# Virtana/robot_camera_calibration

Measured on NVIDIA B200. Metric: BA corner observations/s (residual+Jacobian+normal equations), higher is better.
Workload: dtype f64

## Files before the change

### robot_camera_calibration_b200/csrc/assemble.cu

```cuda
#include "common.cuh"
#include "kernels.h"
#include "model.cuh"

namespace rcc {

template <bool RIG, bool EPASS, bool OWN_IS_VIEW>
struct RowSink {
  using PG = PassGeom<RIG>;
  double* row[2];
  double w;
  __device__ __forceinline__ void put6(int i, int col, const double* v) {
    double2* d = reinterpret_cast<double2*>(row[i] + col);
    d[0] = make_double2(w * v[0], w * v[1]);
    d[1] = make_double2(w * v[2], w * v[3]);
    d[2] = make_double2(w * v[4], w * v[5]);
  }
  __device__ __forceinline__ void shared(int i, const double* js, double r) {
    double2* d = reinterpret_cast<double2*>(row[i] + 6);
    d[0] = make_double2(w * js[0], w * js[1]);
    d[1] = make_double2(w * js[2], w * js[3]);
    d[2] = make_double2(w * js[4], w * js[5]);
    d[3] = make_double2(w * js[6], w * js[7]);
    d[4] = make_double2(w * js[8], w * r);
  }
  __device__ __forceinline__ void marker(int i, const double* jm) {
    if (!OWN_IS_VIEW) put6(i, 0, jm);
    else if (EPASS) put6(i, PG::COL_C, jm);
  }
  __device__ __forceinline__ void view(int i, const double* jv) {
    if (OWN_IS_VIEW) put6(i, 0, jv);
    else if (EPASS) put6(i, PG::COL_C, jv);
  }
  __device__ __forceinline__ void ext(int i, const double* jx) { put6(i, PG::COL_X, jx); }
};

__device__ __forceinline__ void cp_async16(void* smem_dst, const void* gmem_src) {
  const unsigned d = (unsigned)__cvta_generic_to_shared(smem_dst);
  asm volatile("cp.async.ca.shared.global [%0], [%1], 16;" ::"r"(d), "l"(gmem_src) : "memory");
}
__device__ __forceinline__ void cp_async_commit() { asm volatile("cp.async.commit_group;" ::: "memory"); }
__device__ __forceinline__ void cp_async_wait_all() { asm volatile("cp.async.wait_group 0;" ::: "memory"); }

__device__ __forceinline__ void dmma(double (&c)[2], double a, double b) {
  asm volatile("mma.sync.aligned.m8n8k4.row.col.f64.f64.f64.f64 {%0,%1}, {%2}, {%3}, {%0,%1};"
               : "+d"(c[0]), "+d"(c[1])
               : "d"(a), "d"(b));
}

#ifndef RCC_K2_MIN_CTAS
#define RCC_K2_MIN_CTAS 3
#endif
#ifndef RCC_K2_MIN_CTAS_F
#define RCC_K2_MIN_CTAS_F 3
#endif

template <bool RIG, bool EPASS>
struct WarpSmem {
  using PG = PassGeom<RIG>;
  static constexpr int RS = EPASS ? PG::RS_E : PG::RS_F;
  static constexpr int BS = 8 * RS + 2;
  static constexpr int STAGE = PG::BPW * BS;
  static constexpr int CONSTS = STAGE + 2 * PG::BPW * POSEX;
  static constexpr int TOTAL = CONSTS + 2 * POSEX + 16;
};

template <bool RIG, bool EPASS, bool OWN_IS_VIEW, bool LOSS>
__global__ void __launch_bounds__(PassGeom<RIG>::WARPS * 32,
                                  (RIG && EPASS) ? 2 : ((!RIG && !EPASS) ? RCC_K2_MIN_CTAS_F : RCC_K2_MIN_CTAS))
assemble_kernel(const AssembleArgs a) {
  using PG = PassGeom<RIG>;
  using WS = WarpSmem<RIG, EPASS>;
  constexpr int BPW = PG::BPW, RS = WS::RS, BS = WS::BS;
  constexpr int PART = EPASS ? PG::PART_E : PG::PART_F;
  extern __shared__ __align__(16) double smem[];
  const int warp = threadIdx.x >> 5, lane = threadIdx.x & 31;
  const int launch_pos = blockIdx.x * PG::WARPS + warp;
  if (launch_pos >= a.n_chunks) return;
  const int chunk_id = a.chunk_list ? a.chunk_list[launch_pos] : launch_pos;
  double* wsm = smem + warp * WS::TOTAL;
  double* rows = wsm;
  double* stage = wsm + WS::STAGE;
  double* own_x = wsm + WS::CONSTS;
  double* ext_x = own_x + POSEX;
  double* sh = ext_x + POSEX;

  const Chunk ch = a.chunks[chunk_id];
  const int b = lane >> 2;
  const int t = lane & 3;
  const double* oth_table = OWN_IS_VIEW ? a.marker_x : a.view_x;

  {
    const double* src = (OWN_IS_VIEW ? a.view_x : a.marker_x) + (size_t)ch.own * POSEX;
    if (lane < POSEX) own_x[lane] = src[lane];
    if (RIG && lane < POSEX) ext_x[lane] = a.ext_x[(size_t)ch.cam * POSEX + lane];
    if (lane < PG::SP) sh[lane] = a.shared[ch.cam * PG::SP + lane];
    for (int k = lane; k < BPW * BS; k += 32) rows[k] = 0.0;
  }
  auto load_oth = [&](int it) -> int {
    return (lane < BPW && it + lane < ch.count) ? a.oth[(int64_t)ch.start + it + lane] : 0;
  };
  auto issue_stage = [&](int it, int buf, int oth_reg) {
    constexpr int PIECES = BPW * (POSEX / 2);
#pragma unroll
    for (int r = 0; r < PIECES / 32; ++r) {
      const int idx = lane + 32 * r;
      const int q = idx / (POSEX / 2), c = idx - q * (POSEX / 2);
      const int o = __shfl_sync(0xffffffffu, oth_reg, q);
      if (it + q < ch.count)
        cp_async16(stage + (buf * BPW + q) * POSEX + 2 * c, oth_table + (size_t)o * POSEX + 2 * c);
    }
    cp_async_commit();
  };
  int oth_cur = load_oth(0);
  int oth_nxt = load_oth(BPW);
  issue_stage(0, 0, oth_cur);
  double2 px_nxt = make_double2(0.0, 0.0);
  if (b < ch.count) px_nxt = *reinterpret_cast<const double2*>(a.pix + ((int64_t)ch.start + b) * 8 + 2 * t);

  double cAA[2] = {0.0, 0.0}, cAB[2] = {0.0, 0.0}, cBB[2] = {0.0, 0.0};
  double cAX[2] = {0.0, 0.0}, cBX[2] = {0.0, 0.0}, cXX[2] = {0.0, 0.0};
  double cost_acc = 0.0;
  double* my_rows = rows + b * BS + t * RS;
  const double* frag = rows + (lane & 3) * RS + (lane >> 2);
  int buf = 0;

  for (int it = 0; it < ch.count; it += BPW, buf ^= 1) {
    const bool valid = (it + b) < ch.count;
    const int64_t g = (int64_t)ch.start + it + b;
    cp_async_wait_all();
    __syncwarp();
    const double2 px = px_nxt;
    if (it + BPW < ch.count) {
      issue_stage(it + BPW, buf ^ 1, oth_nxt);
      oth_nxt = load_oth(it + 2 * BPW);
      if (it + BPW + b < ch.count) px_nxt = *reinterpret_cast<const double2*>(a.pix + (g + BPW) * 8 + 2 * t);
    }
    const double* ox_rec = stage + (buf * BPW + b) * POSEX;
    const double* vx = OWN_IS_VIEW ? own_x : ox_rec;
    const double* mx = OWN_IS_VIEW ? ox_rec : own_x;
    BlockGeom<RIG> geo;
    double ox = 0.0, oy = 0.0;
    if (valid) {
      block_geometry<RIG>(vx, mx, RIG ? ext_x : nullptr, geo);
      corner_xy(t, mx[PX_HS], ox, oy);
    }
    double w = 1.0;
    if (LOSS) {
      double s_blk = 0.0;
      if (valid) {
        CornerRows<RIG> c;
        eval_corner<RIG, false>(geo, sh, ox, oy, px.x, px.y, c);
        s_blk = c.r[0] * c.r[0] + c.r[1] * c.r[1];
      }
      s_blk += __shfl_xor_sync(0xffffffffu, s_blk, 1);
      s_blk += __shfl_xor_sync(0xffffffffu, s_blk, 2);
      double rho1;
      const double rho = robust_rho(a.loss, a.loss_a2, s_blk, rho1);
      w = sqrt(rho1);
      if (EPASS && valid && t == 0) cost_acc += rho;
    }
    if (valid) {
      RowSink<RIG, EPASS, OWN_IS_VIEW> sink{{my_rows, my_rows + 4 * RS}, w};
      double r0, r1;
      const double depth = eval_corner_emit<RIG>(geo, sh, ox, oy, px.x, px.y, sink, r0, r1);
      if (!(depth > 0.0) || !isfinite(r0) || !isfinite(r1)) *a.fail_flag = 1;
    }
    __syncwarp();
    auto block_products = [&](int bb) {
      const double* f0 = frag + bb * BS;
      const double* f1 = f0 + 4 * RS;
      const double a0 = f0[0], a1 = f1[0];
      const double b0 = f0[PG::COL_B], b1 = f1[PG::COL_B];
      dmma(cAA, a0, a0); dmma(cAA, a1, a1);
      dmma(cAB, a0, b0); dmma(cAB, a1, b1);
      if (EPASS) { dmma(cBB, b0, b0); dmma(cBB, b1, b1); }
      if (RIG) {
        const double x0 = f0[PG::COL_X], x1 = f1[PG::COL_X];
        dmma(cAX, a0, x0); dmma(cAX, a1, x1);
        if (EPASS) {
          dmma(cBX, b0, x0); dmma(cBX, b1, x1);
          dmma(cXX, x0, x0); dmma(cXX, x1, x1);
        }
      }
      if (EPASS) {
        const double t0 = f0[PG::COL_C], t1 = f1[PG::COL_C];
        double cW[2] = {0.0, 0.0};
        dmma(cW, a0, t0); dmma(cW, a1, t1);
        if (lane < 24 && (lane & 3) < 3)
          *reinterpret_cast<double2*>(a.W + ((int64_t)ch.start + it + bb) * 36 + (lane >> 2) * 6 + 2 * (lane & 3)) =
              make_double2(cW[0], cW[1]);
      }
    };
    if (ch.count - it >= BPW) {
#pragma unroll
      for (int bb = 0; bb < BPW; ++bb) block_products(bb);
    } else {
#pragma unroll 1
      for (int bb = 0; bb < ch.count - it; ++bb) block_products(bb);
    }
    __syncwarp();
  }

  double2* out = reinterpret_cast<double2*>(a.partials + (size_t)chunk_id * PART) + lane;
  if (EPASS) {
    out[TE_AA * 32] = make_double2(cAA[0], cAA[1]);
    out[TE_AB * 32] = make_double2(cAB[0], cAB[1]);
    out[TE_BB * 32] = make_double2(cBB[0], cBB[1]);
    if (RIG) {
      out[TE_AX * 32] = make_double2(cAX[0], cAX[1]);
      out[TE_BX * 32] = make_double2(cBX[0], cBX[1]);
      out[TE_XX * 32] = make_double2(cXX[0], cXX[1]);
    }
    if (LOSS) {
#pragma unroll
      for (int o = 16; o > 0; o >>= 1) cost_acc += __shfl_xor_sync(0xffffffffu, cost_acc, o);
    }
    if (lane == 0) a.partials[(size_t)chunk_id * PART + PG::TILES_E * 64] = cost_acc;
  } else {
    out[TF_AA * 32] = make_double2(cAA[0], cAA[1]);
    out[TF_AB * 32] = make_double2(cAB[0], cAB[1]);
    if (RIG) out[TF_AX * 32] = make_double2(cAX[0], cAX[1]);
  }
}

template <bool RIG, bool EPASS, bool OWN_IS_VIEW, bool LOSS>
static void launch_assemble_t(const AssembleArgs& a, cudaStream_t s) {
  using PG = PassGeom<RIG>;
  if (a.n_chunks == 0) return;
  const size_t smem = PG::WARPS * WarpSmem<RIG, EPASS>::TOTAL * sizeof(double);
  auto k = assemble_kernel<RIG, EPASS, OWN_IS_VIEW, LOSS>;
  static SmemOptIn optin;
  optin.ensure(k, smem);
  const int grid = ceil_div(a.n_chunks, PG::WARPS);
  k<<<grid, PG::WARPS * 32, smem, s>>>(a);
  RCC_CUDA(cudaGetLastError());
}

template <bool LOSS>
static void launch_assemble_l(bool rig, bool epass, bool own_is_view, const AssembleArgs& a, cudaStream_t s) {
  const int sel = (rig ? 4 : 0) | (epass ? 2 : 0) | (own_is_view ? 1 : 0);
  switch (sel) {
    case 0: launch_assemble_t<false, false, false, LOSS>(a, s); break;
    case 1: launch_assemble_t<false, false, true, LOSS>(a, s); break;
    case 2: launch_assemble_t<false, true, false, LOSS>(a, s); break;
    case 3: launch_assemble_t<false, true, true, LOSS>(a, s); break;
    case 4: launch_assemble_t<true, false, false, LOSS>(a, s); break;
    case 5: launch_assemble_t<true, false, true, LOSS>(a, s); break;
    case 6: launch_assemble_t<true, true, false, LOSS>(a, s); break;
    default: launch_assemble_t<true, true, true, LOSS>(a, s); break;
  }
}

// ... 218 lines not shown
```

### robot_camera_calibration_b200/csrc/evaluate.cu

```cuda
#include "common.cuh"
#include "kernels.h"
#include "model.cuh"

namespace rcc {

constexpr int EVAL_THREADS = 256;
constexpr int EVAL_CTAS_PER_SM = 2;

int eval_grid(int64_t n) {
  const int64_t groups = (n + 7) / 8;
  return (int)std::max<int64_t>(1, std::min<int64_t>((groups + EVAL_THREADS / 32 - 1) / (EVAL_THREADS / 32),
                                                     (int64_t)NUM_SMS_B200 * EVAL_CTAS_PER_SM));
}

__device__ __forceinline__ double block_sum(double v, double* red) {
#pragma unroll
  for (int o = 16; o > 0; o >>= 1) v += __shfl_xor_sync(0xffffffffu, v, o);
  const int warp = threadIdx.x >> 5, lane = threadIdx.x & 31;
  if (lane == 0) red[warp] = v;
  __syncthreads();
  double s = 0.0;
  if (threadIdx.x == 0) {
    for (int w = 0; w < (int)(blockDim.x >> 5); ++w) s += red[w];
  }
// ... 92 lines not shown
  }
  const double s = block_sum(cost, red);
  if (threadIdx.x == 0 && a.cost2_partials) a.cost2_partials[blockIdx.x] = s;
}

template <bool RIG>
static void launch_evaluate_t(const EvalArgs& a, cudaStream_t s) {
  evaluate_kernel<RIG><<<eval_grid(a.n), EVAL_THREADS, 0, s>>>(a);
  RCC_CUDA(cudaGetLastError());
}

template <bool RIG, bool OWN_IS_VIEW>
struct CeresSink {
  using ER = EvalRec<RIG>;
  double* rec;
  int q, t;
  double d0[5];
  __device__ __forceinline__ void put6(int off, int i, const double* v) {
    double2* d = reinterpret_cast<double2*>(rec + off + q * 48 + (2 * t + i) * 6);
    d[0] = make_double2(v[0], v[1]);
    d[1] = make_double2(v[2], v[3]);
    d[2] = make_double2(v[4], v[5]);
  }
  __device__ __forceinline__ void shared(int i, const double* js, double r) {
    double2* d = reinterpret_cast<double2*>(rec + ER::JI + q * 32 + (2 * t + i) * 4);
    d[0] = make_double2(js[0], js[1]);
    d[1] = make_double2(js[2], js[3]);
    rec[ER::RES + q * 8 + 2 * t + i] = r;
    if (i == 0) {
#pragma unroll
      for (int k = 0; k < 5; ++k) d0[k] = js[4 + k];
    } else {
      d = reinterpret_cast<double2*>(rec + ER::JD + q * 40 + 10 * t);
      d[0] = make_double2(d0[0], d0[1]);
      d[1] = make_double2(d0[2], d0[3]);
      d[2] = make_double2(d0[4], js[4]);
      d[3] = make_double2(js[5], js[6]);
      d[4] = make_double2(js[7], js[8]);
    }
  }
  __device__ __forceinline__ void marker(int i, const double* jm) { put6(ER::JM, i, jm); }
  __device__ __forceinline__ void view(int i, const double* jv) { put6(ER::JV, i, jv); }
  __device__ __forceinline__ void ext(int i, const double* jx) { put6(ER::JX, i, jx); }
};

__device__ __forceinline__ void ev_cp_async16(void* smem_dst, const void* gmem_src) {
// ... 187 lines not shown
```

### robot_camera_calibration_b200/csrc/kernels.h

```cpp
#pragma once

#include <cuda_runtime.h>
#include <math.h>
#include <stdint.h>

namespace rcc {

template <bool RIG>
struct PassGeom {
  static constexpr int BPW = 8;
  static constexpr int SP = RIG ? 15 : 9;
  static constexpr int WARPS = 4;
  static constexpr int RS_E = RIG ? 36 : 28;
  static constexpr int RS_F = RIG ? 28 : 20;
  static constexpr int COL_B = 8, COL_X = 16, COL_C = RIG ? 24 : 16;
  static constexpr int TILES_E = RIG ? 6 : 3;
  static constexpr int TILES_F = RIG ? 3 : 2;
  static constexpr int PART_E = TILES_E * 64 + 8;
  static constexpr int PART_F = TILES_F * 64;
};
enum TileE : int { TE_AA = 0, TE_AB = 1, TE_BB = 2, TE_AX = 3, TE_BX = 4, TE_XX = 5 };
enum TileF : int { TF_AA = 0, TF_AB = 1, TF_AX = 2 };

struct Chunk {
  int32_t own;
  int32_t cam;
  int32_t start;
  int32_t count;
};

struct AssembleArgs {
  const int32_t* oth;
  const double* pix;
  const Chunk* chunks;
  int32_t n_chunks;
  const int32_t* chunk_list;
  const double* view_x;
  const double* marker_x;
  const double* ext_x;
  const double* shared;
  double* partials;
  double* W;
  int32_t* fail_flag;
  int32_t loss;
  double loss_a2;
};

void launch_assemble(bool rig, bool epass, bool own_is_view, const AssembleArgs& a, cudaStream_t s);

struct FinalizeSideArgs {
  const double* partials;
  const Chunk* chunks;
  const int32_t* chunk_ptr;
  int32_t n_own;
  int32_t n_shared;
  double* Hoo;
  double* go;
  double* Hos;
};

struct FinalizeSharedArgs {
  const double* part_e;
  const int32_t* cam_chunks_e;
  const int32_t* cam_ptr_e;
  int32_t n_cam;
  int32_t n_shared;
  double* Hss;
  double* gs;
// ... 209 lines not shown
```

### robot_camera_calibration_b200/csrc/model.cuh

```cuda
#pragma once

#include <math.h>

#if defined(__CUDACC__)
#define RCC_HD __host__ __device__ __forceinline__
#else
#define RCC_HD inline
#endif

namespace rcc {

constexpr int POSEX = 24;
constexpr int PX_R = 0, PX_JR = 9, PX_T = 18;
constexpr int PX_RJ = PX_JR;
constexpr int PX_HS = 21;

RCC_HD double sinc_d(double t2, double t) {
  if (t2 < 1e-6) return 1.0 - t2 * (1.0 / 6.0) + t2 * t2 * (1.0 / 120.0);
  return sin(t) / t;
}

RCC_HD void expand_pose(const double* __restrict__ p, double* __restrict__ o) {
  const double x = p[0], y = p[1], z = p[2];
  const double t2 = x * x + y * y + z * z;
// ... 199 lines not shown
  if (!RIG) {
    a_cross(A, P, 1.0, B);
#pragma unroll
    for (int i = 0; i < 2; ++i) row_mat(B[i], g.Jrv, out.jv[i]);
  } else {
    double qb[3], Ax[2][3];
#pragma unroll
    for (int i = 0; i < 3; ++i) qb[i] = g.Rbm[3 * i] * ox + g.Rbm[3 * i + 1] * oy + g.qb0[i];
#pragma unroll
    for (int i = 0; i < 2; ++i) {
      row_mat(A[i], g.RxT, Ax[i]);
#pragma unroll
      for (int j = 0; j < 3; ++j) out.jx[i][3 + j] = -Ax[i][j];
    }
    a_cross(Ax, qb, 1.0, B);
#pragma unroll
    for (int i = 0; i < 2; ++i) row_mat(B[i], g.Jrv, out.jv[i]);
    a_cross(A, P, 1.0, B);
#pragma unroll
    for (int i = 0; i < 2; ++i) row_mat(B[i], g.Jrx, out.jx[i]);
  }
}

template <bool RIG, class Geo, class Sink>
RCC_HD double eval_corner_emit(const Geo& g, const double* __restrict__ sh, double ox, double oy,
                               double pu, double pv, Sink& sink, double& r0, double& r1) {
  const double fx = sh[0], fy = sh[1], cx = sh[2], cy = sh[3];
  const double k1 = sh[4], k2 = sh[5], p1 = sh[6], p2 = sh[7], k3 = sh[8];
  double d[3], P[3];
#pragma unroll
  for (int i = 0; i < 3; ++i) {
    d[i] = g.Rcm[3 * i] * ox + g.Rcm[3 * i + 1] * oy;
    P[i] = d[i] + g.c0[i];
  }
  const double iz = 1.0 / P[2];
  const double x = P[0] * iz, y = P[1] * iz;
  const double xx = x * x, yy = y * y, xy = x * y;
  const double r2 = xx + yy;
  const double r4 = r2 * r2, r6 = r4 * r2;
  const double rad = 1.0 + k1 * r2 + k2 * r4 + k3 * r6;
  const double tx = 2.0 * xy, ax = r2 + 2.0 * xx, ay = r2 + 2.0 * yy;
  const double xd = x * rad + p1 * tx + p2 * ax;
  const double yd = y * rad + p1 * ay + p2 * tx;
  r0 = fx * xd + cx - pu;
  r1 = fy * yd + cy - pv;
  {
    const double fxx = fx * x, fyy = fy * y;
    const double js0[9] = {xd, 0.0, 1.0, 0.0, fxx * r2, fxx * r4, fx * tx, fx * ax, fxx * r6};
    sink.shared(0, js0, r0);
    const double js1[9] = {0.0, yd, 0.0, 1.0, fyy * r2, fyy * r4, fy * ay, fy * tx, fyy * r6};
    sink.shared(1, js1, r1);
  }
  const double drad = k1 + 2.0 * k2 * r2 + 3.0 * k3 * r4;
  const double dxx = rad + 2.0 * xx * drad + 2.0 * p1 * y + 6.0 * p2 * x;
  const double dxy = 2.0 * xy * drad + 2.0 * p1 * x + 2.0 * p2 * y;
  const double dyy = rad + 2.0 * yy * drad + 6.0 * p1 * y + 2.0 * p2 * x;
  double A[2][3];
  A[0][0] = fx * dxx * iz;
  A[0][1] = fx * dxy * iz;
  A[0][2] = -(A[0][0] * x + A[0][1] * y);
  A[1][0] = fy * dxy * iz;
  A[1][1] = fy * dyy * iz;
  A[1][2] = -(A[1][0] * x + A[1][1] * y);

  double jvt[2][3];
  double B[2][3];
  a_cross(A, d, -1.0, B);
#pragma unroll
  for (int i = 0; i < 2; ++i) {
    double jm[6];
    row_mat(B[i], g.Km, jm);
#pragma unroll
    for (int j = 0; j < 3; ++j) {
      const double mt = A[i][0] * g.Mt[j] + A[i][1] * g.Mt[3 + j] + A[i][2] * g.Mt[6 + j];
      jm[3 + j] = mt;
// ... 65 lines not shown
```

### robot_camera_calibration_b200/csrc/problem.cu

```cuda
#include "problem.h"
#include "model.cuh"

#include <nvtx3/nvToolsExt.h>
#include <omp.h>
#include <string.h>

#include <algorithm>
#include <cmath>
#include <cstdlib>
#include <numeric>
#include <tuple>
#include <type_traits>

using namespace rcc;

#define RCC_STR2(x) #x
#define RCC_STR(x) RCC_STR2(x)

namespace rcc {

static const char* kStageNames[ST_COUNT] = {"expand", "assemble_e", "assemble_f", "finalize", "schur_prep",
                                            "schur_syrk", "schur_shared", "allreduce", "mask", "cholesky",
                                            "backsub", "cost", "evaluate", "h2d", "inverse", "covariance",
                                            "cov_extract"};
// ... 274 lines not shown
#pragma omp parallel for
      for (int64_t i = 0; i < n; ++i) group[i] = piece_of_e[e_of[perm_f[i]]];
    }
    make_chunks(perm_f, seg_f, cam_idx, P->n_f, bpw, ch_max, chunks, chunk_ptr, P->pix_identity ? &group : nullptr);
    std::vector<int32_t> plist;
    plist.reserve(chunks.size());
    for (int k = 0; k < rcc_ba_problem::PIX_PIECES; ++k) {
      P->f_piece_ptr[k] = (int)plist.size();
      if (P->pix_identity)
        for (size_t c = 0; c < chunks.size(); ++c)
          if (group[chunks[c].start] == k) plist.push_back((int32_t)c);
    }
    P->f_piece_ptr[rcc_ba_problem::PIX_PIECES] = (int)plist.size();
    if (plist.empty()) plist.push_back(0);
    P->f_piece_list.upload(plist, s);
  }
  P->n_chunks_f = (int)chunks.size();
  P->f_chunks.upload(chunks, s);
  P->f_chunk_ptr.upload(chunk_ptr, s);
  cam_lists(chunks, P->n_cam, list, ptr);
  P->cam_chunks_f.upload(list, s);
  P->cam_ptr_f.upload(ptr, s);
  {
    std::vector<int32_t> oth((size_t)n);
#pragma omp parallel for
    for (int64_t i = 0; i < n; ++i) oth[i] = e_of[perm_f[i]];
    P->f_oth.upload(oth, s);
    std::vector<int32_t> e_pos_of_caller((size_t)n), f_inv((size_t)n);
#pragma omp parallel for
    for (int64_t i = 0; i < n; ++i) e_pos_of_caller[perm_e[i]] = (int32_t)i;
#pragma omp parallel for
    for (int64_t i = 0; i < n; ++i) f_inv[e_pos_of_caller[perm_f[i]]] = (int32_t)i;
    P->f_inv.upload(f_inv, s);
    RCC_CUDA(cudaStreamSynchronize(s));
  }

  std::vector<int32_t> row_ptr((size_t)P->n_e + 1, 0), pair_e, pair_f, pair_mptr, members;
  pair_e.reserve((size_t)n);
  pair_f.reserve((size_t)n);
  pair_mptr.reserve((size_t)n + 1);
  members.reserve((size_t)n);
  {
    std::vector<std::pair<int32_t, int32_t>> tmp;
    for (int e = 0; e < P->n_e; ++e) {
      tmp.clear();
      for (int pos = seg_e[e]; pos < seg_e[e + 1]; ++pos) tmp.emplace_back(f_of[perm_e[pos]], pos);
      if (P->n_cam > 1) std::sort(tmp.begin(), tmp.end());
      for (size_t k = 0; k < tmp.size(); ++k) {
        if (k == 0 || tmp[k].first != tmp[k - 1].first) {
          pair_e.push_back(e);
// ... 73 lines not shown
      P->syrk_grp_cta[0] = 0;
      P->syrk_grp_col[0] = 0;
      int64_t cum = 0;
      int g = 1;
      for (int J = 0; J < nct && g < G; ++J) {
        cum += std::min(P->n_f, (J + 1) * ctw);
        if (cum * G >= (int64_t)order.size() * g) {
          P->syrk_grp_cta[g] = (int)cum;
          P->syrk_grp_col[g] = std::min(6 * P->n_f, (J + 1) * ctw * 6);
          ++g;
        }
      }
      for (; g <= rcc_ba_problem::SYRK_GROUPS; ++g) {
        P->syrk_grp_cta[g] = (int)order.size();
        P->syrk_grp_col[g] = 6 * P->n_f;
      }
    }
    if (cta_list.empty()) cta_list.assign(2, 0);
    P->syrk_ctas.upload(cta_list, s);
    RCC_CUDA(cudaStreamSynchronize(s));
  }

  P->e_pix.alloc((size_t)n * 8);
  P->f_pix.alloc((size_t)n * 8);
  P->part_e.alloc((size_t)P->n_chunks_e * (P->rig ? PassGeom<true>::PART_E : PassGeom<false>::PART_E));
  P->part_f.alloc((size_t)P->n_chunks_f * (P->rig ? PassGeom<true>::PART_F : PassGeom<false>::PART_F));
  P->W.alloc((size_t)n * 36);
  P->Y.alloc((size_t)std::max<int64_t>(P->n_pairs, 1) * 36);
  P->cost_partials.alloc((size_t)std::max(std::max(1, eval_grid(n)), P->n_chunks_e));
  RCC_CUDA(cudaStreamSynchronize(s));
  P->have_obs = true;
  P->linearized = P->schur_done = P->step_ready = P->cand_ready = false;
}

static void refresh_constants(P_t* P) {
  if (!P->const_dirty) return;
  const std::vector<uint8_t>& ce = P->elim_view ? P->c_view : P->c_marker;
  const std::vector<uint8_t>& cf = P->elim_view ? P->c_marker : P->c_view;
  P->e_const.upload(ce, P->stream);
  std::vector<int32_t> idx;
  for (int f = 0; f < P->n_f; ++f)
    if (cf[f])
      for (int k = 0; k < 6; ++k) idx.push_back(6 * f + k);
  for (int c = 0; c < P->n_cam; ++c) {
    const int b = 6 * P->n_f + c * P->sp;
    if (P->c_intr[c]) for (int k = 0; k < 4; ++k) idx.push_back(b + k);
    if (P->c_dist[c]) for (int k = 4; k < 9; ++k) idx.push_back(b + k);
// ... 13 lines not shown
                      P->n_cam, P->sp, P->ext_x.p, P->stream);
  P->expanded_valid = true;
}

static void ensure_pixels(P_t* P) {
  if (!P->pix_pending) return;
  for (int k = 0; k < rcc_ba_problem::PIX_PIECES; ++k) RCC_CUDA(cudaStreamWaitEvent(P->stream, P->ev_piece[k], 0));
  P->pix_pending = false;
}

static void do_linearize(P_t* P) {
  RCC_REQUIRE(P->have_obs, RCC_NOT_READY, "set_observations has not been called");
  ensure_expanded(P);
  RCC_CUDA(cudaMemsetAsync(P->fail_flag.p, 0, sizeof(int32_t), P->stream));
  AssembleArgs a{};
  bool f_done = false;
  a.view_x = P->view_x.p;
  a.marker_x = P->marker_x.p;
  a.ext_x = P->ext_x.p;
  a.shared = P->shared.p;
  a.fail_flag = P->fail_flag.p;
  a.loss = P->loss;
  a.loss_a2 = P->loss_scale * P->loss_scale;
  {
    Scoped t(P, ST_ASSEMBLE_E, P->pix_pending ? 0 : 1);
    a.oth = P->e_oth.p;
    a.pix = P->e_pix.p;
    a.chunks = P->e_chunks.p;
    a.n_chunks = P->n_chunks_e;
    a.partials = P->part_e.p;
    a.W = P->W.p;
    if (P->pix_pending) {
      const int part = P->rig ? PassGeom<true>::PART_E : PassGeom<false>::PART_E;
      f_done = P->n_obs >= rcc_ba_problem::LARGE_UPLOAD_BLOCKS;
      for (int k = 0; k < rcc_ba_problem::PIX_PIECES; ++k) {
        const int c0 = P->piece_chunk[k], c1 = P->piece_chunk[k + 1];
        RCC_CUDA(cudaStreamWaitEvent(P->stream, P->ev_piece[k], 0));
        if (c1 <= c0) continue;
        AssembleArgs ak = a;
        ak.chunks = P->e_chunks.p + c0;
        ak.n_chunks = c1 - c0;
        ak.partials = P->part_e.p + (size_t)c0 * part;
        launch_assemble(P->rig, true, P->elim_view, ak, P->stream);
        P->launch_count += 1;
        if (!f_done) continue;
        AssembleArgs af = a;
// ... 627 lines not shown
  sum.allreduce_ms = m[ST_ALLREDUCE];
  sum.solve_ms = m[ST_MASK] + m[ST_CHOLESKY];
  sum.backsub_ms = m[ST_BACKSUB];
  sum.cost_ms = m[ST_COST];
  P->timer.on = was_on;
}

template <typename T>
static void load_pixels(P_t* P, const T* pixels, bool piecewise) {
  if (piecewise) {
    constexpr bool f64 = std::is_same<T, double>::value;
    if (!f64) P->staging.ensure((size_t)P->n_obs * 8 * sizeof(T));
    T* dst = f64 ? reinterpret_cast<T*>(P->e_pix.p) : reinterpret_cast<T*>(P->staging.p);
    Scoped t(P, ST_H2D, 0);
    RCC_CUDA(cudaEventRecord(P->ev_fork, P->stream));
    RCC_CUDA(cudaStreamWaitEvent(P->side_stream, P->ev_fork, 0));
    RCC_CUDA(cudaStreamWaitEvent(P->side_stream2, P->ev_fork, 0));
    for (int k = 0; k < rcc_ba_problem::PIX_PIECES; ++k) {
      cudaStream_t cs = (k & 1) ? P->side_stream2 : P->side_stream;
      const int64_t b0 = P->piece_block[k], b1 = P->piece_block[k + 1];
      if (b1 > b0) {
        RCC_CUDA(cudaMemcpyAsync(dst + b0 * 8, pixels + b0 * 8, (size_t)(b1 - b0) * 8 * sizeof(T),
                                 cudaMemcpyHostToDevice, cs));
        launch_load_pixels<T>(f64 ? nullptr : dst + b0 * 8, nullptr, P->e_pix.p + b0 * 8, P->f_inv.p + b0, P->f_pix.p,
                              b1 - b0, cs);
        P->launch_count += 1;
      }
      RCC_CUDA(cudaEventRecord(P->ev_piece[k], cs));
    }
    P->pix_pending = true;
  } else {
    const size_t bytes = (size_t)P->n_obs * 8 * sizeof(T);
    Scoped t(P, ST_H2D, P->n_obs > 0 ? 1 : 0);
    P->staging.ensure(bytes);
    if (bytes) RCC_CUDA(cudaMemcpyAsync(P->staging.p, pixels, bytes, cudaMemcpyHostToDevice, P->stream));
    launch_load_pixels<T>(reinterpret_cast<const T*>(P->staging.p), P->e_orig.p, P->e_pix.p, P->f_inv.p, P->f_pix.p,
                          P->n_obs, P->stream);
  }
}

template <typename T>
static void set_observations(P_t* P, const int32_t* view_idx, const int32_t* marker_idx, const int32_t* cam_idx,
                             const T* pixels) {
  RCC_REQUIRE(view_idx && marker_idx && pixels, RCC_BAD_ARG, "null pointer");
  build_indices(P, view_idx, marker_idx, cam_idx);
  load_pixels(P, pixels, false);
  RCC_CUDA(cudaStreamSynchronize(P->stream));
  P->staging.release();
}
// ... 53 lines not shown
  try {
    int ndev = 0;
    cudaError_t ce = cudaGetDeviceCount(&ndev);
    if (ce != cudaSuccess || ndev == 0)
      throw Error(RCC_CUDA_ERROR, std::string("no CUDA device: ") + cudaGetErrorString(ce) +
                                      " (this library has no CPU fallback)");
    RCC_REQUIRE(opt->device >= 0 && opt->device < ndev, RCC_BAD_ARG, "device ordinal out of range");
    RCC_CUDA(cudaSetDevice(opt->device));
    cudaDeviceProp prop;
    RCC_CUDA(cudaGetDeviceProperties(&prop, opt->device));
    RCC_REQUIRE(prop.major == 10, RCC_CUDA_ERROR,
                std::string("device is sm_") + std::to_string(prop.major * 10 + prop.minor) +
                    "; this library carries sm_100a code only");
    P->opt = *opt;
    P->rig = opt->model == RCC_MODEL_RIG;
    P->sp = P->rig ? 15 : 9;
    P->n_cam = opt->n_cameras;
    P->n_shared = P->n_cam * P->sp;
    P->fin_slices = fin_slices(prop.multiProcessorCount, P->n_cam);
    P->n_views = opt->n_views;
    P->n_markers = opt->n_markers;
    P->n_obs = opt->n_obs_blocks;
    P->elim_view = opt->eliminate == RCC_ELIM_VIEWS || (opt->eliminate == RCC_ELIM_AUTO && opt->n_views >= opt->n_markers);
    P->n_e = P->elim_view ? P->n_views : P->n_markers;
    P->n_f = P->elim_view ? P->n_markers : P->n_views;
    P->n_bb = (P->n_shared + 1 + 5) / 6;
    P->n_red = 6 * P->n_f + P->n_shared;
    P->ld = 6 * P->n_f + 6 * P->n_bb;
    RCC_REQUIRE((int64_t)P->n_red * P->ld < (int64_t)1 << 40, RCC_BAD_ARG, "reduced system too large");
    RCC_REQUIRE(P->n_bb * 6 <= 128, RCC_BAD_ARG,
                "too many cameras: the shared border holds at most 125 parameters (8 rig or 13 single-model cameras)");
    RCC_CUDA(cudaStreamCreateWithFlags(&P->stream, cudaStreamNonBlocking));
    P->own_stream = true;
    RCC_CUDA(cudaStreamCreateWithFlags(&P->side_stream, cudaStreamNonBlocking));
    RCC_CUDA(cudaStreamCreateWithFlags(&P->side_stream2, cudaStreamNonBlocking));
    RCC_CUDA(cudaEventCreateWithFlags(&P->ev_fork, cudaEventDisableTiming));
    RCC_CUDA(cudaEventCreateWithFlags(&P->ev_join, cudaEventDisableTiming));
    for (auto& e : P->ev_piece) RCC_CUDA(cudaEventCreateWithFlags(&e, cudaEventDisableTiming));
    RCC_CUDA(cudaMallocHost(&P->h_pinned, 64 * sizeof(double)));
    cudaStream_t s = P->stream;
    P->views.alloc((size_t)P->n_views * 6); P->views.zero(s);
    P->views_c.alloc((size_t)P->n_views * 6); P->views_c.zero(s);
    P->markers.alloc((size_t)P->n_markers * 6); P->markers.zero(s);
    P->markers_c.alloc((size_t)P->n_markers * 6); P->markers_c.zero(s);
    P->sizes.alloc((size_t)P->n_markers); P->sizes.zero(s);
    P->shared.alloc((size_t)P->n_shared); P->shared.zero(s);
// ... 683 lines not shown
```

### robot_camera_calibration_b200/csrc/problem.h

```cpp
#pragma once

#include <cublas_v2.h>
#include <cusolverDn.h>
#include <nccl.h>

#include <map>
#include <string>
#include <vector>

#include "common.cuh"
#include "dense.h"
#include "kernels.h"

namespace rcc {

enum Stage : int {
  ST_EXPAND = 0, ST_ASSEMBLE_E, ST_ASSEMBLE_F, ST_FINALIZE, ST_SCHUR_PREP, ST_SCHUR_SYRK, ST_SCHUR_SHARED,
  ST_ALLREDUCE, ST_MASK, ST_CHOLESKY, ST_BACKSUB, ST_COST, ST_EVALUATE, ST_H2D, ST_INVERSE, ST_COVARIANCE,
  ST_COV_EXTRACT, ST_COUNT
};
const char* stage_name(int s);

struct StageTimer {
  struct Pending { int stage; cudaEvent_t a, b; };
// ... 32 lines not shown
  int n_chunks_e = 0, n_chunks_f = 0;
  cudaStream_t stream = nullptr;
  bool own_stream = false;
  cudaStream_t side_stream = nullptr, side_stream2 = nullptr;
  cudaEvent_t ev_fork = nullptr, ev_join = nullptr;
  static constexpr int PIX_PIECES = 8;
  static constexpr int64_t LARGE_UPLOAD_BLOCKS = 4000000;
  bool pix_identity = false;
  bool pix_pending = false;
  int piece_chunk[PIX_PIECES + 1] = {0};
  int64_t piece_block[PIX_PIECES + 1] = {0};
  cudaEvent_t ev_piece[PIX_PIECES] = {nullptr};
  std::string err;
  int64_t launch_count = 0;

  rcc::DBuf<double> views, markers, sizes, shared, views_c, markers_c, shared_c;
  rcc::DBuf<double> view_x, marker_x, ext_x, view_xc, marker_xc, ext_xc;
  bool expanded_valid = false;
  std::vector<uint8_t> c_view, c_marker, c_intr, c_dist, c_ext;
  bool const_dirty = true;

  rcc::DBuf<int32_t> e_own, e_oth, e_cam, e_orig, f_oth, f_inv, e_chunk_ptr, f_chunk_ptr;
  rcc::DBuf<double> e_pix, f_pix;
  rcc::DBuf<char> staging;
  rcc::DBuf<rcc::Chunk> e_chunks, f_chunks;
  rcc::DBuf<int32_t> cam_chunks_e, cam_ptr_e, cam_chunks_f, cam_ptr_f;
  rcc::DBuf<int32_t> f_piece_list;
  int f_piece_ptr[PIX_PIECES + 1] = {0};
  std::vector<int32_t> row_ptr_h;
  rcc::DBuf<int32_t> row_ptr, pair_e, pair_f, pair_mptr, pair_members, row_pos0, col_ptr, col_pair, tile_ptr, syrk_ctas, e_count;
  rcc::DBuf<uint8_t> e_const;

  rcc::DBuf<double> fin_scratch, part_e, part_f, W, Hee, ge, Hes, Hff, gf, Hfs, Hss, gs, cost2_cam;
  rcc::DBuf<double> Linv, Y, Yb, d2e, S, shared_scratch, rhs, d2f, gFm, delta_F, delta_e, bs_partials, stats;
  rcc::DBuf<int32_t> const_idx, fail_flag, fin_done;
  int n_const = 0;
  double radius_used = 0.0;
  rcc::DBuf<double> o_res, o_ji, o_jd, o_jv, o_jm, o_jx, cost_partials, scalar;

  cusolverDnHandle_t solver = nullptr;
  cublasHandle_t blas = nullptr;
  rcc::DBuf<double> potrf_work, packed_S;
  rcc::DBuf<int> dev_info;
  int potrf_lwork = 0;
  rcc::DBuf<double> cov_e, cov_f, cov_s, cov_diag;
  rcc::DBuf<int32_t> cov_info;
// ... 27 lines not shown
```

### robot_camera_calibration_b200/csrc/schur.cu

```cuda
#include "common.cuh"
#include "kernels.h"

namespace rcc {

constexpr int PREP_REC = 38;
__global__ void __launch_bounds__(128, 3) schur_prep_kernel(const SchurPrepArgs a) {
  const int e = (blockIdx.x * blockDim.x + threadIdx.x) >> 5;
  const int lane = threadIdx.x & 31;
  if (e >= a.n_e) return;
  double L[6][6], Li[6][6], d2[6];
  const double* H = a.Hee + (size_t)e * 36;
  const bool is_const = a.e_const[e] != 0;
#pragma unroll
  for (int i = 0; i < 6; ++i) {
    const double dg = H[i * 6 + i];
    d2[i] = lm_diagonal(dg, a.radius, a.min_diag, a.max_diag, a.jacobi);
  }
#pragma unroll
  for (int i = 0; i < 6; ++i)
#pragma unroll
    for (int j = 0; j < 6; ++j) {
      L[i][j] = 0.0;
      Li[i][j] = 0.0;
    }
// ... 1035 lines not shown
  return make_double2((double)v.x, (double)v.y);
}
__device__ __forceinline__ double2 load_corner(const int16_t* p) {
  const short2 v = *reinterpret_cast<const short2*>(p);
  return make_double2((double)v.x, (double)v.y);
}

template <typename T>
__global__ void load_pixels_kernel(const T* __restrict__ src, const int32_t* __restrict__ orig,
                                   double* __restrict__ e_pix, const int32_t* __restrict__ f_inv,
                                   double* __restrict__ f_pix, int64_t n) {
  const int64_t i = (int64_t)blockIdx.x * blockDim.x + threadIdx.x;
  if (i >= n * 4) return;
  const int64_t g = i >> 2;
  const int q = (int)(i & 3);
  double2 v;
  if (src) {
    const int64_t sg = orig ? (int64_t)orig[g] : g;
    v = load_corner(src + sg * 8 + q * 2);
    reinterpret_cast<double2*>(e_pix + g * 8)[q] = v;
  } else {
    v = reinterpret_cast<const double2*>(e_pix + g * 8)[q];
  }
  reinterpret_cast<double2*>(f_pix + (int64_t)f_inv[g] * 8)[q] = v;
}
template <typename T>
void launch_load_pixels(const T* src, const int32_t* orig, double* e_pix, const int32_t* f_inv, double* f_pix,
                        int64_t n, cudaStream_t s) {
  if (n == 0) return;
  load_pixels_kernel<T><<<ceil_div(n * 4, 256), 256, 0, s>>>(src, orig, e_pix, f_inv, f_pix, n);
  RCC_CUDA(cudaGetLastError());
}
template void launch_load_pixels(const double*, const int32_t*, double*, const int32_t*, double*, int64_t, cudaStream_t);
template void launch_load_pixels(const int32_t*, const int32_t*, double*, const int32_t*, double*, int64_t, cudaStream_t);
template void launch_load_pixels(const int16_t*, const int32_t*, double*, const int32_t*, double*, int64_t, cudaStream_t);

__global__ void fill_kernel(double* p, int64_t n, double v) {
  for (int64_t i = (int64_t)blockIdx.x * blockDim.x + threadIdx.x; i < n; i += (int64_t)gridDim.x * blockDim.x) p[i] = v;
}
void launch_fill(double* p, int64_t n, double v, cudaStream_t s) {
  fill_kernel<<<NUM_SMS_B200 * 8, 256, 0, s>>>(p, n, v);
  RCC_CUDA(cudaGetLastError());
}

__global__ void __launch_bounds__(256) fp64_peak_kernel(double* out, int iters) {
  double a0 = threadIdx.x * 1e-9, a1 = a0 + 1, a2 = a0 + 2, a3 = a0 + 3, a4 = a0 + 4, a5 = a0 + 5, a6 = a0 + 6,
         a7 = a0 + 7;
// ... 20 lines not shown
```

Measured before the change: 11.18 billion.

## Reuse E-pass corner records in F-pass instead of recomputing geometry

In the non-rig, views-eliminated case, the E-pass assembly now writes a compact per-corner record (rotated-marker terms, normalized point, residuals and loss weight) into a buffer ordered by F position. The F-pass reads these records with plain vector loads and rebuilds only the marker and shared Jacobian columns, skipping the cp.async staging of the other pose, the block geometry and the full corner evaluation, including the loss pre-pass. This trades recomputation for extra global writes in the E-pass and an extra record buffer, and removes the F-pass pixel copy and other-index table. The E and F passes must stay ordered and their records consistent.

```diff
diff --git a/robot_camera_calibration_b200/csrc/assemble.cu b/robot_camera_calibration_b200/csrc/assemble.cu
--- a/robot_camera_calibration_b200/csrc/assemble.cu
+++ b/robot_camera_calibration_b200/csrc/assemble.cu
@@ -9,6 +9,10 @@
   using PG = PassGeom<RIG>;
   double* row[2];
   double w;
+  static constexpr int COL_PT = 24;
+  __device__ __forceinline__ void point(double x, double y) {
+    if (!RIG && EPASS && OWN_IS_VIEW) *reinterpret_cast<double2*>(row[0] + COL_PT) = make_double2(x, y);
+  }
   __device__ __forceinline__ void put6(int i, int col, const double* v) {
     double2* d = reinterpret_cast<double2*>(row[i] + col);
     d[0] = make_double2(w * v[0], w * v[1]);
@@ -34,6 +38,25 @@
   __device__ __forceinline__ void ext(int i, const double* jx) { put6(i, PG::COL_X, jx); }
 };
 
+struct RecRowSink {
+  double* row[2];
+  double w;
+  __device__ __forceinline__ void marker(int i, const double* rot, const double* tr) {
+    double2* d = reinterpret_cast<double2*>(row[i]);
+    d[0] = make_double2(rot[0], rot[1]);
+    d[1] = make_double2(rot[2], tr[0]);
+    d[2] = make_double2(tr[1], tr[2]);
+  }
+  __device__ __forceinline__ void shared(int i, const double* js, double r) {
+    double2* d = reinterpret_cast<double2*>(row[i] + 6);
+    d[0] = make_double2(w * js[0], w * js[1]);
+    d[1] = make_double2(w * js[2], w * js[3]);
+    d[2] = make_double2(w * js[4], w * js[5]);
+    d[3] = make_double2(w * js[6], w * js[7]);
+    d[4] = make_double2(w * js[8], r);
+  }
+};
+
 __device__ __forceinline__ void cp_async16(void* smem_dst, const void* gmem_src) {
   const unsigned d = (unsigned)__cvta_generic_to_shared(smem_dst);
   asm volatile("cp.async.ca.shared.global [%0], [%1], 16;" ::"r"(d), "l"(gmem_src) : "memory");
@@ -53,25 +76,42 @@
 #ifndef RCC_K2_MIN_CTAS_F
 #define RCC_K2_MIN_CTAS_F 3
 #endif
-
-template <bool RIG, bool EPASS>
+#ifndef RCC_K2_MIN_CTAS_FREC
+#define RCC_K2_MIN_CTAS_FREC 3
+#endif
+
+template <bool RIG, bool EPASS, bool OWN_IS_VIEW>
+constexpr bool uses_records() { return !RIG && EPASS == OWN_IS_VIEW; }
+
+template <bool RIG, bool EPASS, bool STAGED>
 struct WarpSmem {
   using PG = PassGeom<RIG>;
   static constexpr int RS = EPASS ? PG::RS_E : PG::RS_F;
   static constexpr int BS = 8 * RS + 2;
   static constexpr int STAGE = PG::BPW * BS;
-  static constexpr int CONSTS = STAGE + 2 * PG::BPW * POSEX;
+  static constexpr int CONSTS = STAGE + (STAGED ? 2 * PG::BPW * POSEX : 0);
   static constexpr int TOTAL = CONSTS + 2 * POSEX + 16;
 };
 
+template <bool RIG, bool EPASS, bool OWN_IS_VIEW>
+constexpr int min_ctas() {
+  if (RIG) return EPASS ? 2 : RCC_K2_MIN_CTAS;
+  if (EPASS) return RCC_K2_MIN_CTAS;
+  return uses_records<RIG, EPASS, OWN_IS_VIEW>() ? RCC_K2_MIN_CTAS_FREC : RCC_K2_MIN_CTAS_F;
+}
+
 template <bool RIG, bool EPASS, bool OWN_IS_VIEW, bool LOSS>
-__global__ void __launch_bounds__(PassGeom<RIG>::WARPS * 32,
-                                  (RIG && EPASS) ? 2 : ((!RIG && !EPASS) ? RCC_K2_MIN_CTAS_F : RCC_K2_MIN_CTAS))
+__global__ void __launch_bounds__(PassGeom<RIG>::WARPS * 32, min_ctas<RIG, EPASS, OWN_IS_VIEW>())
 assemble_kernel(const AssembleArgs a) {
   using PG = PassGeom<RIG>;
-  using WS = WarpSmem<RIG, EPASS>;
+  constexpr bool REC = uses_records<RIG, EPASS, OWN_IS_VIEW>();
+  constexpr bool FREC = REC && !EPASS;
+  constexpr int RECN = CornerRec::doubles(LOSS);
+  using WS = WarpSmem<RIG, EPASS, !FREC>;
   constexpr int BPW = PG::BPW, RS = WS::RS, BS = WS::BS;
   constexpr int PART = EPASS ? PG::PART_E : PG::PART_F;
+  using Sink = RowSink<RIG, EPASS, OWN_IS_VIEW>;
+  static_assert(!(REC && EPASS) || (PG::COL_C + 8 <= Sink::COL_PT && Sink::COL_PT + 2 <= RS), "record staging outside the pad");
   extern __shared__ __align__(16) double smem[];
   const int warp = threadIdx.x >> 5, lane = threadIdx.x & 31;
   const int launch_pos = blockIdx.x * PG::WARPS + warp;
@@ -111,11 +151,32 @@
     }
     cp_async_commit();
   };
-  int oth_cur = load_oth(0);
-  int oth_nxt = load_oth(BPW);
-  issue_stage(0, 0, oth_cur);
+  auto load_rec = [&](int64_t g, double2 (&q)[RECN / 2]) {
+    const double2* src = reinterpret_cast<const double2*>(a.rec + g * 4 * RECN + 2 * t);
+#pragma unroll
+    for (int k = 0; k < RECN / 2; ++k) q[k] = __ldg(src + 4 * k);
+  };
+  int oth_nxt = 0;
   double2 px_nxt = make_double2(0.0, 0.0);
-  if (b < ch.count) px_nxt = *reinterpret_cast<const double2*>(a.pix + ((int64_t)ch.start + b) * 8 + 2 * t);
+  double2 rec_nxt[RECN / 2];
+  double pt[3], RJ[9];
+  if (FREC) {
+#pragma unroll
+    for (int k = 0; k < RECN / 2; ++k) rec_nxt[k] = make_double2(0.0, 0.0);
+    if (b < ch.count) load_rec((int64_t)ch.start + b, rec_nxt);
+    __syncwarp();
+    double ox, oy;
+    corner_xy(t, own_x[PX_HS], ox, oy);
+#pragma unroll
+    for (int i = 0; i < 3; ++i) pt[i] = own_x[PX_R + 3 * i] * ox + own_x[PX_R + 3 * i + 1] * oy;
+#pragma unroll
+    for (int i = 0; i < 9; ++i) RJ[i] = own_x[PX_RJ + i];
+  } else {
+    const int oth_cur = load_oth(0);
+    oth_nxt = load_oth(BPW);
+    issue_stage(0, 0, oth_cur);
+    if (b < ch.count) px_nxt = *reinterpret_cast<const double2*>(a.pix + ((int64_t)ch.start + b) * 8 + 2 * t);
+  }
 
   double cAA[2] = {0.0, 0.0}, cAB[2] = {0.0, 0.0}, cBB[2] = {0.0, 0.0};
   double cAX[2] = {0.0, 0.0}, cBX[2] = {0.0, 0.0}, cXX[2] = {0.0, 0.0};
@@ -127,45 +188,65 @@
   for (int it = 0; it < ch.count; it += BPW, buf ^= 1) {
     const bool valid = (it + b) < ch.count;
     const int64_t g = (int64_t)ch.start + it + b;
-    cp_async_wait_all();
+    if (FREC) {
+      double2 q[RECN / 2];
+#pragma unroll
+      for (int k = 0; k < RECN / 2; ++k) q[k] = rec_nxt[k];
+      if (it + BPW + b < ch.count) load_rec(g + BPW, rec_nxt);
+      if (valid) {
+        const double* r = reinterpret_cast<const double*>(q);
+        RecRowSink sink{{my_rows, my_rows + 4 * RS}, LOSS ? r[CornerRec::W] : 1.0};
+        double rot[3];
+        marker_rot_world(pt, r + CornerRec::A_U, RJ, rot);
+        sink.marker(0, rot, r + CornerRec::A_U);
+        marker_rot_world(pt, r + CornerRec::A_V, RJ, rot);
+        sink.marker(1, rot, r + CornerRec::A_V);
+        const double x = r[CornerRec::XY], y = r[CornerRec::XY + 1];
+        emit_shared_columns(sh, x, y, distort(sh, x, y), r[CornerRec::R], r[CornerRec::R + 1], sink);
+      }
+    } else {
+      cp_async_wait_all();
+      __syncwarp();
+      const double2 px = px_nxt;
+      if (it + BPW < ch.count) {
+        issue_stage(it + BPW, buf ^ 1, oth_nxt);
+        oth_nxt = load_oth(it + 2 * BPW);
+        if (it + BPW + b < ch.count) px_nxt = *reinterpret_cast<const double2*>(a.pix + (g + BPW) * 8 + 2 * t);
+      }
+      const double* ox_rec = stage + (buf * BPW + b) * POSEX;
+      const double* vx = OWN_IS_VIEW ? own_x : ox_rec;
+      const double* mx = OWN_IS_VIEW ? ox_rec : own_x;
+      BlockGeom<RIG> geo;
+      double ox = 0.0, oy = 0.0;
+      if (valid) {
+        block_geometry<RIG>(vx, mx, RIG ? ext_x : nullptr, geo);
+        corner_xy(t, mx[PX_HS], ox, oy);
+      }
+      double w = 1.0;
+      if (LOSS) {
+        double s_blk = 0.0;
+        if (valid) {
+          CornerRows<RIG> c;
+          eval_corner<RIG, false>(geo, sh, ox, oy, px.x, px.y, c);
+          s_blk = c.r[0] * c.r[0] + c.r[1] * c.r[1];
+        }
+        s_blk += __shfl_xor_sync(0xffffffffu, s_blk, 1);
+        s_blk += __shfl_xor_sync(0xffffffffu, s_blk, 2);
+        double rho1;
+        const double rho = robust_rho(a.loss, a.loss_a2, s_blk, rho1);
+        w = sqrt(rho1);
+        if (EPASS && valid && t == 0) cost_acc += rho;
+        if (REC && valid) my_rows[4 * RS + Sink::COL_PT] = w;
+      }
+      if (valid) {
+        Sink sink{{my_rows, my_rows + 4 * RS}, w};
+        double r0, r1;
+        const double depth = eval_corner_emit<RIG>(geo, sh, ox, oy, px.x, px.y, sink, r0, r1);
+        if (!(depth > 0.0) || !isfinite(r0) || !isfinite(r1)) *a.fail_flag = 1;
+      }
+    }
     __syncwarp();
-    const double2 px = px_nxt;
-    if (it + BPW < ch.count) {
-      issue_stage(it + BPW, buf ^ 1, oth_nxt);
-      oth_nxt = load_oth(it + 2 * BPW);
-      if (it + BPW + b < ch.count) px_nxt = *reinterpret_cast<const double2*>(a.pix + (g + BPW) * 8 + 2 * t);
-    }
-    const double* ox_rec = stage + (buf * BPW + b) * POSEX;
-    const double* vx = OWN_IS_VIEW ? own_x : ox_rec;
-    const double* mx = OWN_IS_VIEW ? ox_rec : own_x;
-    BlockGeom<RIG> geo;
-    double ox = 0.0, oy = 0.0;
-    if (valid) {
-      block_geometry<RIG>(vx, mx, RIG ? ext_x : nullptr, geo);
-      corner_xy(t, mx[PX_HS], ox, oy);
-    }
-    double w = 1.0;
-    if (LOSS) {
-      double s_blk = 0.0;
-      if (valid) {
-        CornerRows<RIG> c;
-        eval_corner<RIG, false>(geo, sh, ox, oy, px.x, px.y, c);
-        s_blk = c.r[0] * c.r[0] + c.r[1] * c.r[1];
-      }
-      s_blk += __shfl_xor_sync(0xffffffffu, s_blk, 1);
-      s_blk += __shfl_xor_sync(0xffffffffu, s_blk, 2);
-      double rho1;
-      const double rho = robust_rho(a.loss, a.loss_a2, s_blk, rho1);
-      w = sqrt(rho1);
-      if (EPASS && valid && t == 0) cost_acc += rho;
-    }
-    if (valid) {
-      RowSink<RIG, EPASS, OWN_IS_VIEW> sink{{my_rows, my_rows + 4 * RS}, w};
-      double r0, r1;
-      const double depth = eval_corner_emit<RIG>(geo, sh, ox, oy, px.x, px.y, sink, r0, r1);
-      if (!(depth > 0.0) || !isfinite(r0) || !isfinite(r1)) *a.fail_flag = 1;
-    }
-    __syncwarp();
+    const int fpos = (REC && EPASS && valid) ? a.f_inv[g] : 0;
     auto block_products = [&](int bb) {
       const double* f0 = frag + bb * BS;
       const double* f1 = f0 + 4 * RS;
@@ -198,6 +279,18 @@
 #pragma unroll 1
       for (int bb = 0; bb < ch.count - it; ++bb) block_products(bb);
     }
+    if (REC && EPASS && valid) {
+      const double* u = my_rows;
+      const double* v = my_rows + 4 * RS;
+      constexpr int AT = PG::COL_C + 3, RC = PG::COL_B + 7;
+      double2* d = reinterpret_cast<double2*>(a.rec + (int64_t)fpos * 4 * RECN + 2 * t);
+      d[0] = make_double2(u[AT], u[AT + 1]);
+      d[4] = make_double2(u[AT + 2], v[AT]);
+      d[8] = make_double2(v[AT + 1], v[AT + 2]);
+      d[12] = *reinterpret_cast<const double2*>(u + Sink::COL_PT);
+      d[16] = make_double2(u[RC], v[RC]);
+      if (LOSS) d[20] = make_double2(v[Sink::COL_PT], 0.0);
+    }
     __syncwarp();
   }
 
@@ -226,8 +319,10 @@
 template <bool RIG, bool EPASS, bool OWN_IS_VIEW, bool LOSS>
 static void launch_assemble_t(const AssembleArgs& a, cudaStream_t s) {
   using PG = PassGeom<RIG>;
+  constexpr bool REC = uses_records<RIG, EPASS, OWN_IS_VIEW>();
   if (a.n_chunks == 0) return;
-  const size_t smem = PG::WARPS * WarpSmem<RIG, EPASS>::TOTAL * sizeof(double);
+  RCC_REQUIRE(!REC || (a.rec && (!EPASS || a.f_inv)), RCC_BAD_ARG, "assemble: corner records not provided");
+  const size_t smem = PG::WARPS * WarpSmem<RIG, EPASS, !(REC && !EPASS)>::TOTAL * sizeof(double);
   auto k = assemble_kernel<RIG, EPASS, OWN_IS_VIEW, LOSS>;
   static SmemOptIn optin;
   optin.ensure(k, smem);
diff --git a/robot_camera_calibration_b200/csrc/evaluate.cu b/robot_camera_calibration_b200/csrc/evaluate.cu
--- a/robot_camera_calibration_b200/csrc/evaluate.cu
+++ b/robot_camera_calibration_b200/csrc/evaluate.cu
@@ -138,6 +138,7 @@
     d[1] = make_double2(v[2], v[3]);
     d[2] = make_double2(v[4], v[5]);
   }
+  __device__ __forceinline__ void point(double, double) {}
   __device__ __forceinline__ void shared(int i, const double* js, double r) {
     double2* d = reinterpret_cast<double2*>(rec + ER::JI + q * 32 + (2 * t + i) * 4);
     d[0] = make_double2(js[0], js[1]);
diff --git a/robot_camera_calibration_b200/csrc/kernels.h b/robot_camera_calibration_b200/csrc/kernels.h
--- a/robot_camera_calibration_b200/csrc/kernels.h
+++ b/robot_camera_calibration_b200/csrc/kernels.h
@@ -21,6 +21,11 @@
 };
 enum TileE : int { TE_AA = 0, TE_AB = 1, TE_BB = 2, TE_AX = 3, TE_BX = 4, TE_XX = 5 };
 enum TileF : int { TF_AA = 0, TF_AB = 1, TF_AX = 2 };
+
+struct CornerRec {
+  static constexpr int A_U = 0, A_V = 3, XY = 6, R = 8, W = 10;
+  static constexpr int doubles(bool loss) { return loss ? 12 : 10; }
+};
 
 struct Chunk {
   int32_t own;
@@ -44,6 +49,8 @@
   int32_t* fail_flag;
   int32_t loss;
   double loss_a2;
+  const int32_t* f_inv;
+  double* rec;
 };
 
 void launch_assemble(bool rig, bool epass, bool own_is_view, const AssembleArgs& a, cudaStream_t s);
diff --git a/robot_camera_calibration_b200/csrc/model.cuh b/robot_camera_calibration_b200/csrc/model.cuh
--- a/robot_camera_calibration_b200/csrc/model.cuh
+++ b/robot_camera_calibration_b200/csrc/model.cuh
@@ -245,6 +245,39 @@
   }
 }
 
+struct Distorted {
+  double xx, yy, xy, r2, r4, r6, rad, tx, ax, ay, xd, yd;
+};
+RCC_HD Distorted distort(const double* __restrict__ sh, double x, double y) {
+  const double k1 = sh[4], k2 = sh[5], p1 = sh[6], p2 = sh[7], k3 = sh[8];
+  Distorted q;
+  q.xx = x * x; q.yy = y * y; q.xy = x * y;
+  q.r2 = q.xx + q.yy;
+  q.r4 = q.r2 * q.r2; q.r6 = q.r4 * q.r2;
+  q.rad = 1.0 + k1 * q.r2 + k2 * q.r4 + k3 * q.r6;
+  q.tx = 2.0 * q.xy; q.ax = q.r2 + 2.0 * q.xx; q.ay = q.r2 + 2.0 * q.yy;
+  q.xd = x * q.rad + p1 * q.tx + p2 * q.ax;
+  q.yd = y * q.rad + p1 * q.ay + p2 * q.tx;
+  return q;
+}
+
+template <class Sink>
+RCC_HD void emit_shared_columns(const double* __restrict__ sh, double x, double y, const Distorted& q, double r0,
+                                double r1, Sink& sink) {
+  const double fx = sh[0], fy = sh[1];
+  const double fxx = fx * x, fyy = fy * y;
+  const double js0[9] = {q.xd, 0.0, 1.0, 0.0, fxx * q.r2, fxx * q.r4, fx * q.tx, fx * q.ax, fxx * q.r6};
+  sink.shared(0, js0, r0);
+  const double js1[9] = {0.0, q.yd, 0.0, 1.0, fyy * q.r2, fyy * q.r4, fy * q.ay, fy * q.tx, fyy * q.r6};
+  sink.shared(1, js1, r1);
+}
+
+RCC_HD void marker_rot_world(const double* __restrict__ p, const double* __restrict__ aw, const double* __restrict__ RJ,
+                             double* __restrict__ out) {
+  const double c[3] = {p[1] * aw[2] - p[2] * aw[1], p[2] * aw[0] - p[0] * aw[2], p[0] * aw[1] - p[1] * aw[0]};
+  row_mat(c, RJ, out);
+}
+
 template <bool RIG, class Geo, class Sink>
 RCC_HD double eval_corner_emit(const Geo& g, const double* __restrict__ sh, double ox, double oy,
                                double pu, double pv, Sink& sink, double& r0, double& r1) {
@@ -258,22 +291,12 @@
   }
   const double iz = 1.0 / P[2];
   const double x = P[0] * iz, y = P[1] * iz;
-  const double xx = x * x, yy = y * y, xy = x * y;
-  const double r2 = xx + yy;
-  const double r4 = r2 * r2, r6 = r4 * r2;
-  const double rad = 1.0 + k1 * r2 + k2 * r4 + k3 * r6;
-  const double tx = 2.0 * xy, ax = r2 + 2.0 * xx, ay = r2 + 2.0 * yy;
-  const double xd = x * rad + p1 * tx + p2 * ax;
-  const double yd = y * rad + p1 * ay + p2 * tx;
-  r0 = fx * xd + cx - pu;
-  r1 = fy * yd + cy - pv;
-  {
-    const double fxx = fx * x, fyy = fy * y;
-    const double js0[9] = {xd, 0.0, 1.0, 0.0, fxx * r2, fxx * r4, fx * tx, fx * ax, fxx * r6};
-    sink.shared(0, js0, r0);
-    const double js1[9] = {0.0, yd, 0.0, 1.0, fyy * r2, fyy * r4, fy * ay, fy * tx, fyy * r6};
-    sink.shared(1, js1, r1);
-  }
+  sink.point(x, y);
+  const Distorted q = distort(sh, x, y);
+  const double xx = q.xx, yy = q.yy, xy = q.xy, r2 = q.r2, r4 = q.r4, rad = q.rad;
+  r0 = fx * q.xd + cx - pu;
+  r1 = fy * q.yd + cy - pv;
+  emit_shared_columns(sh, x, y, q, r0, r1, sink);
   const double drad = k1 + 2.0 * k2 * r2 + 3.0 * k3 * r4;
   const double dxx = rad + 2.0 * xx * drad + 2.0 * p1 * y + 6.0 * p2 * x;
   const double dxy = 2.0 * xy * drad + 2.0 * p1 * x + 2.0 * p2 * y;
diff --git a/robot_camera_calibration_b200/csrc/problem.cu b/robot_camera_calibration_b200/csrc/problem.cu
--- a/robot_camera_calibration_b200/csrc/problem.cu
+++ b/robot_camera_calibration_b200/csrc/problem.cu
@@ -320,10 +320,15 @@
   P->cam_chunks_f.upload(list, s);
   P->cam_ptr_f.upload(ptr, s);
   {
-    std::vector<int32_t> oth((size_t)n);
+    if (P->f_records) {
+      P->f_oth.release();
+    } else {
+      std::vector<int32_t> oth((size_t)n);
 #pragma omp parallel for
-    for (int64_t i = 0; i < n; ++i) oth[i] = e_of[perm_f[i]];
-    P->f_oth.upload(oth, s);
+      for (int64_t i = 0; i < n; ++i) oth[i] = e_of[perm_f[i]];
+      P->f_oth.upload(oth, s);
+      RCC_CUDA(cudaStreamSynchronize(s));
+    }
     std::vector<int32_t> e_pos_of_caller((size_t)n), f_inv((size_t)n);
 #pragma omp parallel for
     for (int64_t i = 0; i < n; ++i) e_pos_of_caller[perm_e[i]] = (int32_t)i;
@@ -443,7 +448,12 @@
   }
 
   P->e_pix.alloc((size_t)n * 8);
-  P->f_pix.alloc((size_t)n * 8);
+  if (P->f_records) {
+    P->f_pix.release();
+    P->f_rec.alloc((size_t)n * 4 * CornerRec::doubles(P->loss != 0));
+  } else {
+    P->f_pix.alloc((size_t)n * 8);
+  }
   P->part_e.alloc((size_t)P->n_chunks_e * (P->rig ? PassGeom<true>::PART_E : PassGeom<false>::PART_E));
   P->part_f.alloc((size_t)P->n_chunks_f * (P->rig ? PassGeom<true>::PART_F : PassGeom<false>::PART_F));
   P->W.alloc((size_t)n * 36);
@@ -503,6 +513,11 @@
   a.fail_flag = P->fail_flag.p;
   a.loss = P->loss;
   a.loss_a2 = P->loss_scale * P->loss_scale;
+  if (P->f_records) {
+    P->f_rec.ensure((size_t)P->n_obs * 4 * CornerRec::doubles(P->loss != 0));
+    a.f_inv = P->f_inv.p;
+    a.rec = P->f_rec.p;
+  }
   {
     Scoped t(P, ST_ASSEMBLE_E, P->pix_pending ? 0 : 1);
     a.oth = P->e_oth.p;
@@ -1176,9 +1191,11 @@
       if (b1 > b0) {
         RCC_CUDA(cudaMemcpyAsync(dst + b0 * 8, pixels + b0 * 8, (size_t)(b1 - b0) * 8 * sizeof(T),
                                  cudaMemcpyHostToDevice, cs));
-        launch_load_pixels<T>(f64 ? nullptr : dst + b0 * 8, nullptr, P->e_pix.p + b0 * 8, P->f_inv.p + b0, P->f_pix.p,
-                              b1 - b0, cs);
-        P->launch_count += 1;
+        if (!f64 || P->f_pix.p) {
+          launch_load_pixels<T>(f64 ? nullptr : dst + b0 * 8, nullptr, P->e_pix.p + b0 * 8, P->f_inv.p + b0, P->f_pix.p,
+                                b1 - b0, cs);
+          P->launch_count += 1;
+        }
       }
       RCC_CUDA(cudaEventRecord(P->ev_piece[k], cs));
     }
@@ -1278,6 +1295,7 @@
     P->n_markers = opt->n_markers;
     P->n_obs = opt->n_obs_blocks;
     P->elim_view = opt->eliminate == RCC_ELIM_VIEWS || (opt->eliminate == RCC_ELIM_AUTO && opt->n_views >= opt->n_markers);
+    P->f_records = !P->rig && P->elim_view;
     P->n_e = P->elim_view ? P->n_views : P->n_markers;
     P->n_f = P->elim_view ? P->n_markers : P->n_views;
     P->n_bb = (P->n_shared + 1 + 5) / 6;
diff --git a/robot_camera_calibration_b200/csrc/problem.h b/robot_camera_calibration_b200/csrc/problem.h
--- a/robot_camera_calibration_b200/csrc/problem.h
+++ b/robot_camera_calibration_b200/csrc/problem.h
@@ -78,6 +78,8 @@
 
   rcc::DBuf<int32_t> e_own, e_oth, e_cam, e_orig, f_oth, f_inv, e_chunk_ptr, f_chunk_ptr;
   rcc::DBuf<double> e_pix, f_pix;
+  bool f_records = false;
+  rcc::DBuf<double> f_rec;
   rcc::DBuf<char> staging;
   rcc::DBuf<rcc::Chunk> e_chunks, f_chunks;
   rcc::DBuf<int32_t> cam_chunks_e, cam_ptr_e, cam_chunks_f, cam_ptr_f;
diff --git a/robot_camera_calibration_b200/csrc/schur.cu b/robot_camera_calibration_b200/csrc/schur.cu
--- a/robot_camera_calibration_b200/csrc/schur.cu
+++ b/robot_camera_calibration_b200/csrc/schur.cu
@@ -1081,7 +1081,7 @@
   } else {
     v = reinterpret_cast<const double2*>(e_pix + g * 8)[q];
   }
-  reinterpret_cast<double2*>(f_pix + (int64_t)f_inv[g] * 8)[q] = v;
+  if (f_pix) reinterpret_cast<double2*>(f_pix + (int64_t)f_inv[g] * 8)[q] = v;
 }
 template <typename T>
 void launch_load_pixels(const T* src, const int32_t* orig, double* e_pix, const int32_t* f_inv, double* f_pix,
```

Measured after the change: 11.62 billion (median of 6 runs). +3.9%, better.
